# nz0001na/MorphGANformer

Hardware: AMD Instinct MI355X
Metric: latent-projection iters/sec @1024^2, k=17 latents (higher is better)
Workload: dtype f32; 1 GPU; configs[1]: single 1024x1024 face per GPU, Wing+LPIPS(squeeze)+MSE literal-mode projection step, noise_mode=random, seeded synthetic weights/targets/landmarks; k=17, z_dim=32, targets_per_gpu=1, parallelism=pair-sharded x1, graph_replay=True, loss_generator_overlap=True, steps_per_forward=32

## Files before the change

include/mgf.h:

```cpp
#ifndef MGF_H_
#define MGF_H_

#include <stdint.h>

#ifdef __cplusplus
extern "C" {
#endif

typedef void* mgf_stream_t;

enum { MGF_OK = 0, MGF_EINVAL = -1, MGF_EUNSUPPORTED = -2, MGF_ELAUNCH = -3, MGF_ETOOBIG = -4 };
enum { MGF_F32 = 0, MGF_F64 = 1, MGF_F16 = 2 };
enum { MGF_FILTER_SEPARABLE = 2 };
enum { MGF_FILTER_LARGE = 4 };
enum { MGF_ACT_LINEAR = 1, MGF_ACT_RELU = 2, MGF_ACT_LRELU = 3, MGF_ACT_TANH = 4, MGF_ACT_SIGMOID = 5,
       MGF_ACT_ELU = 6, MGF_ACT_SELU = 7, MGF_ACT_SOFTPLUS = 8, MGF_ACT_SWISH = 9,
       MGF_ACT_RELU_POST = 10 };

const char* mgf_last_error(void);
int mgf_version(void);
int mgf_device_ok(void);

int mgf_bias_act(void* y, const void* x, const void* b, const void* xref, const void* yref, const void* dy,
                 int dtype, int64_t numel, int64_t step_b, int64_t size_b,
// ... 70 lines not shown
                              mgf_stream_t stream);
int mgf_conv3x3_winograd3_f32(float* y, const float* x, const float* u, const float* in_scale, const float* out_scale, int32_t n,
                              int32_t cin, int32_t h, int32_t w, int32_t cout, int32_t out_scale_stride, const mgf_epilogue* ep,
                              mgf_stream_t stream);
int mgf_conv3x3_winograd3_slice_f32(float* y, const float* x, const float* u, const float* in_scale, const float* out_scale, int32_t n,
                                    int32_t cin, int32_t h, int32_t w, int32_t cout, int32_t out_scale_stride, int64_t y_batch,
                                    int32_t y_choff, const mgf_epilogue* ep, mgf_stream_t stream);
int mgf_conv1x1_f32(float* y, const float* x, const float* w, const float* in_scale, int32_t n, int32_t cin, int32_t hw, int32_t cout,
                    int32_t cout_pad, int64_t y_batch, int32_t y_choff, const mgf_epilogue* ep, mgf_stream_t stream);
int mgf_conv1x1_force_shape(int32_t channel_blocks);

int mgf_conv3x3s2_few_inputs_f32(float* y, const float* x, const float* w, const float* bias, int32_t n, int32_t cin, int32_t in_h,
                                 int32_t in_w, int32_t cout, int32_t relu, mgf_stream_t stream);
int mgf_tconv3x3s2_few_outputs_f32(float* y, const float* x, const float* wp, int32_t n, int32_t cin, int32_t h, int32_t w, int32_t cout,
                                   int32_t cout_pad, int32_t pitch, int64_t y_plane, int64_t y_batch, mgf_stream_t stream);
int mgf_conv3x3_winograd3_up2res_f32(float* y, const float* x, const float* u, const float* in_scale, const float* out_scale,
                                     const float* residual_low, int32_t n, int32_t cin, int32_t h, int32_t w, int32_t cout,
                                     int32_t out_scale_stride, const mgf_epilogue* ep, mgf_stream_t stream);
int mgf_winograd3_force_shape(int32_t shape);
int mgf_conv3x3_winograd3_rgb_f32(float* rgb_out, const float* x, const float* u, const float* in_scale, const float* out_scale,
                                  const float* rgb_w, const float* rgb_bias, int32_t n, int32_t cin, int32_t h, int32_t w, int32_t cout,
                                  int32_t out_scale_stride, int32_t rgb_channels, mgf_stream_t stream);
int mgf_conv3x3_winograd_f32(float* y, const float* x, const float* u, const float* in_scale, const float* out_scale, int32_t n,
                             int32_t cin, int32_t h, int32_t w, int32_t cout, int32_t out_scale_stride, const mgf_epilogue* ep,
                             mgf_stream_t stream);

int mgf_tconv3x3s2_border_f32(float* t, const float* x, const float* wp, const float* in_scale, const float* out_scale, int32_t n,
                              int32_t cin, int32_t h, int32_t w, int32_t cout, int32_t cout_pad, int64_t t_pitch, int64_t t_plane,
                              int64_t t_batch, int64_t out_scale_stride, mgf_stream_t stream);

int mgf_tconv3x3s2_winograd_f32(float* t, const float* x, const float* u, const float* in_scale, const float* out_scale, int32_t n,
                                int32_t cin, int32_t h, int32_t w, int32_t cout, int32_t pitch, int64_t t_plane, int64_t t_batch,
                                int64_t out_scale_stride, mgf_stream_t stream);
int mgf_tconv_winograd_weights_f32(float* u, const float* w, int32_t cout, int32_t cin, double gain, mgf_stream_t stream);

int mgf_pack_conv_weights(float* wp, float* wsq, const float* w, int32_t cout, int32_t cin, int32_t kh, int32_t kw,
                          int32_t cout_pad, float gain, int32_t flip, mgf_stream_t stream);

typedef struct mgf_style_job {
    const float* aff_w;
    const float* aff_b;
    const float* wsq;
    float* s;
    float* d;
    int32_t cin, cout;
    int32_t w_offset;
    float aff_gain, style_gain;
} mgf_style_job;
int mgf_demod_f32(float* d, const float* s, const float* wsq, int32_t n, int32_t cin, int32_t cout, mgf_stream_t stream);
int mgf_demod_bwd_f32(float* ds, const float* dd, const float* d, const float* s, const float* wsq, int32_t n, int32_t cin, int32_t cout,
                      mgf_stream_t stream);
int mgf_style_demod(const mgf_style_job* job, const float* ws, int64_t ws_stride_n, int32_t n, int32_t wdim, mgf_stream_t stream);
int mgf_style_demod_multi(const mgf_style_job* jobs_dev, int32_t njobs, const float* ws, int64_t ws_stride_n,
                          int32_t n, int32_t wdim, int32_t max_cin, mgf_stream_t stream);

int mgf_duplex_attention(float* y, const float* x, const float* wqc, const float* spos, const float* vwb,
                         int32_t n, int32_t c, int32_t f, int32_t t,
                         const mgf_epilogue* ep, int32_t ep_w, float* probs, int32_t* argmax, mgf_stream_t stream);

int mgf_att_map_upsample_f32(float* out, const float* probs, int32_t n, int32_t side, int32_t t, int32_t out_res, int32_t layer,
                             int32_t n_layers, mgf_stream_t stream);

typedef struct mgf_attn_job {
    const float* wmv;
    const float* bmv;
    float* vwb;
// ... 196 lines not shown
```

morphganformer_amd/_lib.py:

```python
from __future__ import annotations

import ctypes as C
import os

import torch

HERE = os.path.dirname(os.path.abspath(__file__))
LIB_PATH = os.environ.get("MGF_LIB_PATH") or os.path.join(HERE, "libmgf_hip.so")

MGF_F32, MGF_F64, MGF_F16 = 0, 1, 2
ACT_IDS = {"linear": 1, "relu": 2, "lrelu": 3, "tanh": 4, "sigmoid": 5, "elu": 6, "selu": 7, "softplus": 8, "swish": 9,
           "relu_post": 10}
MAX_TAPS = 9

i32, i64, f32, f64, vp = C.c_int32, C.c_int64, C.c_float, C.c_double, C.c_void_p


class Epilogue(C.Structure):
    _fields_ = [("bias", vp), ("noise", vp), ("noise_strength", vp), ("noise_n", i32), ("act", i32), ("alpha", f32),
                ("gain", f32), ("residual", vp)]


class ConvDesc(C.Structure):
    _fields_ = [("n", i32), ("cin", i32), ("in_h", i32), ("in_w", i32), ("cout", i32), ("cout_pad", i32),
# ... 12 lines not shown
    _fields_ = [("aff_w", vp), ("aff_b", vp), ("wsq", vp), ("s", vp), ("d", vp), ("cin", i32), ("cout", i32),
                ("w_offset", i32), ("aff_gain", f32), ("style_gain", f32)]


class AttnJob(C.Structure):
    _fields_ = [("wmv", vp), ("bmv", vp), ("vwb", vp), ("c", i32), ("w_offset", i32)]


class StyleBwdJob(C.Structure):
    _fields_ = [("aff_w", vp), ("wsq", vp), ("s", vp), ("d", vp), ("ds_part", vp), ("dc_part", vp), ("cin", i32), ("cout", i32),
                ("s_chunks", i32), ("d_chunks", i32), ("aff_gain", f32), ("style_gain", f32)]


class AttnGradJob(C.Structure):
    _fields_ = [("dg", vp), ("probs", vp), ("dc", vp), ("cpre", vp), ("part", vp), ("dvwb", vp), ("dc_part", vp), ("c", i32), ("f", i32),
                ("slices", i32), ("nchunk", i32), ("blk_grad", i32), ("blk_dot", i32), ("blk_red", i32), ("pad_", i32)]


class AttnBwdJob(C.Structure):
    _fields_ = [("wmv", vp), ("dvwb", vp), ("c", i32), ("pad_", i32)]


_SIGS = {
    "mgf_last_error": (C.c_char_p, []),
    "mgf_version": (C.c_int, []),
    "mgf_device_ok": (C.c_int, []),
    "mgf_bias_act": (C.c_int, [vp, vp, vp, vp, vp, vp, C.c_int, i64, i64, i64, C.c_int, C.c_int, f32, f32, f32, vp]),
    "mgf_upfirdn2d": (C.c_int, [vp, vp, vp, C.c_int, i32, i32, i32, i32, i64, i64, i64, i64, i32, i32, i64, i64, i64, i64,
                                i32, i32, i32, i32, i32, i32, i32, i32, i32, i32, i32, f32, C.POINTER(Epilogue), vp]),
    "mgf_conv_taps_f32": (C.c_int, [vp, vp, vp, vp, vp, C.POINTER(ConvDesc), C.POINTER(Epilogue), vp]),
    "mgf_conv_taps_bf16x3_f32": (C.c_int, [vp, vp, vp, vp, vp, C.POINTER(ConvDesc), C.POINTER(Epilogue), vp]),
    "mgf_tconv3x3s2_border_f32": (C.c_int, [vp, vp, vp, vp, vp, i32, i32, i32, i32, i32, i32, i64, i64, i64, i64, vp]),
    "mgf_tconv3x3s2_winograd_f32": (C.c_int, [vp, vp, vp, vp, vp, i32, i32, i32, i32, i32, i32, i64, i64, i64, vp]),
    "mgf_tconv_winograd_weights_f32": (C.c_int, [vp, vp, i32, i32, C.c_double, vp]),
    "mgf_winograd_weights_f32": (C.c_int, [vp, vp, i32, i32, f32, vp]),
    "mgf_conv3x3_winograd_f32": (C.c_int, [vp, vp, vp, vp, vp, i32, i32, i32, i32, i32, i32, C.POINTER(Epilogue), vp]),
    "mgf_winograd2_weights_f32": (C.c_int, [vp, vp, i32, i32, f32, vp]),
    "mgf_conv3x3_winograd2_f32": (C.c_int, [vp, vp, vp, vp, vp, i32, i32, i32, i32, i32, i32, C.POINTER(Epilogue), vp]),
    "mgf_conv3x3_winograd2_rgb_f32": (C.c_int, [vp, vp, vp, vp, vp, vp, vp, i32, i32, i32, i32, i32, i32, i32, vp]),
    "mgf_conv3x3_winograd3_f32": (C.c_int, [vp, vp, vp, vp, vp, i32, i32, i32, i32, i32, i32, C.POINTER(Epilogue), vp]),
    "mgf_conv1x1_f32": (C.c_int, [vp, vp, vp, vp, i32, i32, i32, i32, i32, i64, i32, C.POINTER(Epilogue), vp]),
    "mgf_conv3x3s2_few_inputs_f32": (C.c_int, [vp, vp, vp, vp, i32, i32, i32, i32, i32, i32, vp]),
    "mgf_tconv3x3s2_few_outputs_f32": (C.c_int, [vp, vp, vp, i32, i32, i32, i32, i32, i32, i32, i64, i64, vp]),
    "mgf_conv1x1_force_shape": (C.c_int, [i32]),
    "mgf_conv3x3_winograd3_slice_f32": (C.c_int, [vp, vp, vp, vp, vp, i32, i32, i32, i32, i32, i32, i64, i32, C.POINTER(Epilogue), vp]),
    "mgf_conv3x3_winograd3_up2res_f32": (C.c_int, [vp, vp, vp, vp, vp, vp, i32, i32, i32, i32, i32, i32, C.POINTER(Epilogue), vp]),
    "mgf_winograd3_force_shape": (C.c_int, [i32]),
    "mgf_conv3x3_winograd3_rgb_f32": (C.c_int, [vp, vp, vp, vp, vp, vp, vp, i32, i32, i32, i32, i32, i32, i32, vp]),
    "mgf_conv3x3_winograd2_slice_f32": (C.c_int, [vp, vp, vp, vp, vp, i32, i32, i32, i32, i32, i32, i64, i32, C.POINTER(Epilogue), vp]),
    "mgf_pack_conv_weights": (C.c_int, [vp, vp, vp, i32, i32, i32, i32, i32, f32, i32, vp]),
    "mgf_conv_profile_begin": (C.c_int, []),
    "mgf_conv_profile_end": (C.c_int, [C.POINTER(ConvProfRec), i32]),
    "mgf_demod_f32": (C.c_int, [vp, vp, vp, i32, i32, i32, vp]),
    "mgf_demod_bwd_f32": (C.c_int, [vp, vp, vp, vp, vp, i32, i32, i32, vp]),
    "mgf_style_demod": (C.c_int, [C.POINTER(StyleJob), vp, i64, i32, i32, vp]),
    "mgf_style_demod_multi": (C.c_int, [vp, i32, vp, i64, i32, i32, i32, vp]),
    "mgf_duplex_attention": (C.c_int, [vp, vp, vp, vp, vp, i32, i32, i32, i32, C.POINTER(Epilogue), i32, vp, vp, vp]),
    "mgf_att_map_upsample_f32": (C.c_int, [vp, vp, i32, i32, i32, i32, i32, i32, vp]),
    "mgf_attn_values": (C.c_int, [C.POINTER(AttnJob), vp, i64, i64, i32, i32, i32, vp]),
    "mgf_attn_values_multi": (C.c_int, [vp, i32, vp, i64, i64, i32, i32, i32, vp]),
    "mgf_randn_f32": (C.c_int, [vp, i64, C.c_uint64, vp, vp]),
    "mgf_rgb_weights_f32": (C.c_int, [vp, vp, vp, i32, i32, i32, vp]),
    "mgf_torgb_compose_weights_f32": (C.c_int, [vp, vp, vp, vp, vp, vp, i32, i32, i32, i32, vp]),
    "mgf_conv3x3_few_outputs_f32": (C.c_int, [vp, vp, vp, vp, i32, i32, i32, i32, i32, vp]),
    "mgf_mapping_param_floats": (i64, [i32, i32, i32]),
    "mgf_mapping_forward": (C.c_int, [vp, vp, vp, i32, i32, i32, i32, i32, vp]),
# ... 138 lines not shown
```

morphganformer_amd/conv.py:

```python
from __future__ import annotations

import ctypes as C
import os
from dataclasses import dataclass

import torch

from . import _lib


def round_up(v: int, m: int) -> int:
    return (v + m - 1) // m * m


def profile_begin():
    _lib.check(_lib.lib().mgf_conv_profile_begin(), "conv_profile_begin")


def profile_end(max_recs=4096):
    recs = (_lib.ConvProfRec * max_recs)()
    n = _lib.lib().mgf_conv_profile_end(recs, max_recs)
    if n < 0:
        _lib.check(n, "conv_profile_end")
    return [(recs[i].kernel.decode(), recs[i].flops, recs[i].seconds, recs[i].ksplit, recs[i].bytes) for i in range(min(n, max_recs))]
# ... 343 lines not shown

def conv3x3s2_few_inputs(x, w, bias=None, relu=False, out=None):
    _lib.require_gpu(x, w, bias, out)
    cout, cin = w.shape[:2]
    assert tuple(w.shape[2:]) == (3, 3) and cin <= 4 and w.is_contiguous() and w.dtype == torch.float32
    assert x.dtype == torch.float32 and x.is_contiguous() and x.shape[1] == cin
    n, _, h, wd = x.shape
    oh, ow = (h - 3) // 2 + 1, (wd - 3) // 2 + 1
    if out is None:
        out = torch.empty([n, cout, oh, ow], dtype=torch.float32, device=x.device)
    assert out.is_contiguous() and tuple(out.shape) == (n, cout, oh, ow)
    rc = _lib.lib().mgf_conv3x3s2_few_inputs_f32(out.data_ptr(), x.data_ptr(), w.data_ptr(), _lib.ptr(bias), n, cin, h, wd, cout, int(relu),
                                                 _lib.stream_ptr())
    _lib.check(rc, "conv3x3s2_few_inputs")
    return out


def conv3x3_few_outputs(x, w, bias=None, out=None):
    _lib.require_gpu(x, w, bias, out)
    n, cin, h, wd = x.shape
    cout = w.shape[1]
    assert x.dtype == torch.float32 and x.is_contiguous() and w.dtype == torch.float32 and w.is_contiguous()
    assert tuple(w.shape) == (n, cout, cin, 3, 3) and cout <= 4
    if out is None:
        out = torch.empty([n, cout, h, wd], dtype=torch.float32, device=x.device)
    assert out.is_contiguous() and tuple(out.shape) == (n, cout, h, wd)
    _lib.check(_lib.lib().mgf_conv3x3_few_outputs_f32(out.data_ptr(), x.data_ptr(), w.data_ptr(), _lib.ptr(bias), n, cin, h, wd, cout,
                                                      _lib.stream_ptr()), "conv3x3_few_outputs")
    return out


TCONV_WINO = os.environ.get("MGF_TCONV_WINO", "1") != "0"
TCONV_WINO_MIN_WGS = 4096


def tconv_winograd_weights(w: torch.Tensor, gain: float = 1.0) -> torch.Tensor:
    _lib.require_gpu(w)
    w = w.contiguous().float()
    cout, cin, kh, kw = w.shape
    assert (kh, kw) == (3, 3) and cin % 4 == 0
    u = torch.empty([25, cin // 4, cout, 4], dtype=torch.float32, device=w.device)
    _lib.check(_lib.lib().mgf_tconv_winograd_weights_f32(u.data_ptr(), w.data_ptr(), cout, cin, float(gain), _lib.stream_ptr()),
               "tconv_winograd_weights")
    return u


def tconv_winograd_ok(n, cin, h, w, cout, out, bf=None) -> bool:
    return bool(TCONV_WINO and SPLIT_TCONV_BORDER and bf is None and h % 2 == 0 and w % 2 == 0 and min(h, w) >= TCONV_SPLIT_MIN and cin % 4 == 0 and cout % 32 == 0
                and out.shape[3] % 4 == 0 and out.data_ptr() % 16 == 0
                and n * -(-h // 4) * -(-w // 32) * (cout // 32) >= TCONV_WINO_MIN_WGS)


def tconv3x3s2_forward(x, pc: PackedConv, in_scale=None, out_scale=None, out=None, bf=None, wt=None):
    _lib.require_gpu(x, pc.wp, in_scale, out_scale, out, wt)
    assert pc.kh == 3 and pc.kw == 3 and x.dtype == torch.float32 and x.is_contiguous()
    n, cin, h, w = x.shape
    oh, ow = 2 * h + 1, 2 * w + 1
    if out is None:
        out = torch.empty([n, pc.cout, oh, tconv_pitch(w)], dtype=torch.float32, device=x.device)
    pitch = out.shape[3]
    assert out.is_contiguous() and tuple(out.shape) == (n, pc.cout, oh, pitch) and pitch >= ow and pitch % 4 == 0
    if NARROW_CONV and pc.cout <= 4 and in_scale is None and out_scale is None:
        rc = _lib.lib().mgf_tconv3x3s2_few_outputs_f32(out.data_ptr(), x.data_ptr(), pc.wp.data_ptr(), n, cin, h, w, pc.cout, pc.cout_pad,
                                                       pitch, oh * pitch, pc.cout * oh * pitch, _lib.stream_ptr())
        _lib.check(rc, "tconv3x3s2_few_outputs")
        return out[:, :, :, :ow]
    if wt is not None and tconv_winograd_ok(n, cin, h, w, pc.cout, out, bf):
        assert tuple(wt.shape) == (25, cin // 4, pc.cout, 4)
        os_stride = 0 if out_scale is None else out_scale.stride(0) if out_scale.ndim == 2 else 0
        rc = _lib.lib().mgf_tconv3x3s2_winograd_f32(out.data_ptr(), x.data_ptr(), wt.data_ptr(), _lib.ptr(in_scale), _lib.ptr(out_scale), n, cin, h,
                                                    w, pc.cout, pitch, oh * pitch, pc.cout * oh * pitch, os_stride, _lib.stream_ptr())
        _lib.check(rc, "tconv3x3s2_winograd")
        rc = _lib.lib().mgf_tconv3x3s2_border_f32(out.data_ptr(), x.data_ptr(), pc.wp.data_ptr(), _lib.ptr(in_scale), _lib.ptr(out_scale),
                                                  n, cin, h, w, pc.cout, pc.cout_pad, pitch, oh * pitch, pc.cout * oh * pitch, os_stride,
                                                  _lib.stream_ptr())
        _lib.check(rc, "tconv3x3s2_border")
        return out[:, :, :, :ow]
    split = SPLIT_TCONV_BORDER and min(h, w) >= (TCONV_SPLIT_MIN if n >= 4 else max(TCONV_SPLIT_MIN, 128))
    use_bf = bf is not None and split and w % 32 == 0 and cin % 16 == 0
    os_stride = 0 if out_scale is None else out_scale.stride(0) if out_scale.ndim == 2 else 0
    d = _desc(n, cin, h, w, pc.cout, pc.cout_pad, h if split else h + 1, w if split else w + 1, 1, 2, TCONV_TAPS, TCONV_GROUPS,
              [0, 0, 1, 1], [0, 1, 0, 1], oh, ow, pitch, oh * pitch, pc.cout * oh * pitch, 0, os_stride)
    if use_bf:
        rc = _lib.lib().mgf_conv_taps_bf16x3_f32(out.data_ptr(), x.data_ptr(), bf.data_ptr(), _lib.ptr(in_scale), _lib.ptr(out_scale),
                                                 C.byref(d), None, _lib.stream_ptr())
    else:
        rc = _lib.lib().mgf_conv_taps_f32(out.data_ptr(), x.data_ptr(), pc.wp.data_ptr(), _lib.ptr(in_scale), _lib.ptr(out_scale),
                                          C.byref(d), None, _lib.stream_ptr())
    _lib.check(rc, "conv_taps(tconv)")
    if split:
        rc = _lib.lib().mgf_tconv3x3s2_border_f32(out.data_ptr(), x.data_ptr(), pc.wp.data_ptr(), _lib.ptr(in_scale), _lib.ptr(out_scale),
                                                  n, cin, h, w, pc.cout, pc.cout_pad, pitch, oh * pitch, pc.cout * oh * pitch, os_stride,
                                                  _lib.stream_ptr())
        _lib.check(rc, "tconv3x3s2_border")
    return out[:, :, :, :ow]


def upfirdn_into(y, x, f2d, up=1, pad=(0, 0, 0, 0), gain=1.0, flip=False, epilogue=None, separable=False, down=1):
    _lib.require_gpu(x, y, f2d)
    n, c, h, w = x.shape
    fh, fw = f2d.shape
    px0, px1, py0, py1 = pad
# ... 12 lines not shown
```

morphganformer_amd/csrc/conv_taps.hip:

```cpp
#include "mgf_common.h"
#include <vector>

namespace {

typedef float f32x16 __attribute__((ext_vector_type(16)));
typedef __bf16 bf16x8 __attribute__((ext_vector_type(8)));
typedef unsigned u32x4 __attribute__((ext_vector_type(4)));

constexpr int CK = 8;
constexpr int CKB = 16;
template <int WM, int WN> struct Slots {
    static constexpr int XS = WN == 4 ? 20 : (WN == 3 ? 15 : (WN == 1 ? 19 : 11));
    static constexpr int WS = WM == 2 ? 5 : 3;
};

struct Ones { float v[2048]; constexpr Ones() : v() { for (int i = 0; i < 2048; ++i) v[i] = 1.0f; } };
__device__ const Ones g_ones = Ones();

struct ConvParams {
    float* y;
    const float* x;
    const float* wp;
    const float* in_scale;
    const float* out_scale;
// ... 841 lines not shown

void mgf_prof_external_begin(hipStream_t st, const char* name, double flops, double bytes) {
    if (!g_prof_on) return;
    ProfRec r;
    r.name = name; r.wm = r.wn = r.mode = r.pipe = r.nt = 0; r.ksplit = 1; r.flops = flops; r.bytes = bytes;
    (void)hipEventCreate(&r.e0); (void)hipEventCreate(&r.e1);
    (void)hipEventRecord(r.e0, st);
    g_prof.push_back(r);
}
void mgf_prof_external_end(hipStream_t st) {
    if (g_prof_on && !g_prof.empty()) (void)hipEventRecord(g_prof.back().e1, st);
}

extern "C" int mgf_conv_profile_end(mgf_conv_prof_rec* out, int32_t max_recs) {
    g_prof_on = false;
    int n = 0;
    for (auto& r : g_prof) {
        if (hipEventSynchronize(r.e1) != hipSuccess) { mgf_set_error("conv_profile_end: event sync failed"); return MGF_ELAUNCH; }
        float ms = 0.f;
        (void)hipEventElapsedTime(&ms, r.e0, r.e1);
        if (out && n < max_recs) {
            mgf_conv_prof_rec& o = out[n];
            if (r.name) snprintf(o.kernel, sizeof(o.kernel), "%s", r.name);
            else snprintf(o.kernel, sizeof(o.kernel), "conv_taps_kernel<%d, %d, %d, %s, %d, 0>", r.wm, r.wn, r.mode, r.pipe ? "true" : "false", r.nt);
            o.flops = r.flops; o.bytes = r.bytes; o.seconds = ms * 1e-3; o.ksplit = r.ksplit;
        }
        ++n;
        (void)hipEventDestroy(r.e0); (void)hipEventDestroy(r.e1);
    }
    g_prof.clear();
    return n;
}

constexpr int TB_POS = 64, TB_CK = 32, TB_LINE = TB_POS / 2 + 1, TB_LP = TB_LINE + 1;
__global__ __launch_bounds__(256) void tconv_border_kernel(float* t, const float* x, const float* wp, const float* in_scale,
                                                           const float* out_scale, int cin, int h, int w, int cout, int cout_pad,
                                                           int64_t pitch, int64_t plane, int64_t batch, int64_t os_stride, int col_groups) {
    __shared__ float Ws[3][TB_CK][64];
    __shared__ float Xl[TB_CK][TB_LP];
    const int tid = threadIdx.x, n = blockIdx.z, co0 = blockIdx.y * 64;
    const int lane = tid & 63, l31 = lane & 31, half = lane >> 5, wv = __builtin_amdgcn_readfirstlane(tid >> 6);
    const bool col = (int)blockIdx.x < col_groups;
    const int p0 = (col ? blockIdx.x : blockIdx.x - col_groups) * TB_POS;
    const int npos = col ? 2 * h + 1 : 2 * w;
    const int lim = col ? h : w;
    const int tap0 = col ? 2 : 6, tapstep = col ? 3 : 1;
    const float* xn = x + (int64_t)n * cin * h * w;
    const int64_t hw = (int64_t)h * w;
    constexpr int XR = (TB_CK * TB_LINE + 255) / 256, WR = 3 * TB_CK * 64 / 256;
    int xsrc[XR];
#pragma unroll
    for (int r = 0; r < XR; ++r) {
        const int e = tid + 256 * r, jj = e % TB_LINE;
        const int i = p0 / 2 - 1 + jj;
        xsrc[r] = (e < TB_CK * TB_LINE && i >= 0 && i < lim) ? (col ? i * w + (w - 1) : (h - 1) * w + i) : -1;
    }
    float wreg[WR], xreg[XR];
    auto request = [&](int c0) {
#pragma unroll
        for (int r = 0; r < WR; ++r) {
            const int e = tid + 256 * r, co = e & 63, ci = (e >> 6) % TB_CK, k = e / (64 * TB_CK);
            const int cg = c0 + ci < cin ? c0 + ci : cin - 1, cc = co0 + co < cout_pad ? co0 + co : cout_pad - 1;
            wreg[r] = wp[((int64_t)(tap0 + k * tapstep) * cin + cg) * cout_pad + cc];
        }
#pragma unroll
        for (int r = 0; r < XR; ++r) {
            const int e = tid + 256 * r, ci = e / TB_LINE;
            const int cg = c0 + ci < cin ? c0 + ci : cin - 1;
            xreg[r] = xn[cg * hw + (xsrc[r] >= 0 ? xsrc[r] : 0)] * (in_scale ? in_scale[(int64_t)n * cin + cg] : 1.0f);
        }
    };
    f32x16 acc[2];
#pragma unroll
    for (int m = 0; m < 2; ++m)
#pragma unroll
        for (int r = 0; r < 16; ++r) acc[m][r] = 0.f;
    request(0);
    for (int c0 = 0; c0 < cin; c0 += TB_CK) {
        __syncthreads();
#pragma unroll
        for (int r = 0; r < WR; ++r) {
            const int e = tid + 256 * r, co = e & 63, ci = (e >> 6) % TB_CK, k = e / (64 * TB_CK);
            Ws[k][ci][co] = c0 + ci < cin ? wreg[r] : 0.f;
        }
#pragma unroll
        for (int r = 0; r < XR; ++r) {
            const int e = tid + 256 * r, jj = e % TB_LINE, ci = e / TB_LINE;
            if (e < TB_CK * TB_LINE) Xl[ci][jj] = (c0 + ci < cin && xsrc[r] >= 0) ? xreg[r] : 0.f;
        }
        __syncthreads();
        if (c0 + TB_CK < cin) request(c0 + TB_CK);
        if (wv < 2) {
#pragma unroll 8
            for (int ci = 0; ci < TB_CK; ++ci)
                acc[0] = __builtin_amdgcn_mfma_f32_32x32x2f32(Ws[2 * half][ci][wv * 32 + l31], Xl[ci][l31 + 1 - half], acc[0], 0, 0, 0);
        } else if (wv == 2) {
#pragma unroll 8
            for (int cp = 0; cp < TB_CK / 2; ++cp) {
                const int ci = 2 * cp + half;
                const float bv = Xl[ci][l31 + 1];
                acc[0] = __builtin_amdgcn_mfma_f32_32x32x2f32(Ws[1][ci][l31], bv, acc[0], 0, 0, 0);
                acc[1] = __builtin_amdgcn_mfma_f32_32x32x2f32(Ws[1][ci][32 + l31], bv, acc[1], 0, 0, 0);
            }
        }
    }
    if (wv > 2) return;
    const int q = p0 + 2 * l31 + (wv == 2 ? 1 : 0);
    if (q >= npos) return;
    const int oy = col ? q : 2 * h, ox = col ? 2 * w : q;
    float* tn = t + (int64_t)n * batch + (int64_t)oy * pitch + ox;
#pragma unroll
    for (int m = 0; m < 2; ++m) {
        if (m == 1 && wv != 2) break;
        const int cb = wv == 2 ? m : wv;
#pragma unroll
        for (int r = 0; r < 16; ++r) {
            const int co = co0 + cb * 32 + (r & 3) + 8 * (r >> 2) + 4 * half;
            if (co < cout) tn[(int64_t)co * plane] = acc[m][r] * (out_scale ? out_scale[(int64_t)n * os_stride + co] : 1.0f);
        }
    }
}

extern "C" int mgf_tconv3x3s2_border_f32(float* t, const float* x, const float* wp, const float* in_scale, const float* out_scale,
                                         int32_t n, int32_t cin, int32_t h, int32_t w, int32_t cout, int32_t cout_pad, int64_t t_pitch,
                                         int64_t t_plane, int64_t t_batch, int64_t out_scale_stride, mgf_stream_t stream) {
    MGF_REQUIRE(t && x && wp && n >= 1 && n <= 65535 && cin >= 1 && h >= 1 && w >= 1 && cout >= 1 && cout_pad >= cout, MGF_EINVAL,
                "tconv3x3s2_border: bad arguments");
    MGF_REQUIRE(t_pitch >= 2 * w + 1 && t_plane >= (int64_t)(2 * h + 1) * t_pitch, MGF_EINVAL, "tconv3x3s2_border: output pitch/plane too small");
    const int col_groups = (int)mgf_cdiv(2 * h + 1, TB_POS), row_groups = (int)mgf_cdiv(2 * w, TB_POS);
    hipLaunchKernelGGL(tconv_border_kernel, dim3(col_groups + row_groups, (unsigned)mgf_cdiv(cout, 64), n), dim3(256), 0, (hipStream_t)stream,
                       t, x, wp, in_scale, out_scale, cin, h, w, cout, cout_pad, t_pitch, t_plane, t_batch, out_scale_stride, col_groups);
    MGF_CHECK_LAUNCH("tconv3x3s2_border");
    return MGF_OK;
}

extern "C" int mgf_pack_conv_weights(float* wp, float* wsq, const float* w, int32_t cout, int32_t cin, int32_t kh, int32_t kw,
                                     int32_t cout_pad, float gain, int32_t flip, mgf_stream_t stream) {
    MGF_REQUIRE(wp && w, MGF_EINVAL, "pack_conv_weights: null pointer");
    MGF_REQUIRE(cout >= 1 && cin >= 1 && kh >= 1 && kw >= 1 && kh * kw <= MGF_MAX_TAPS, MGF_EINVAL, "pack_conv_weights: bad shape");
    MGF_REQUIRE(cout_pad >= cout && cout_pad % 32 == 0, MGF_EINVAL, "pack_conv_weights: cout_pad must be a multiple of 32 >= cout");
    const int64_t total = (int64_t)kh * kw * cin * cout_pad;
    hipLaunchKernelGGL(pack_weights_kernel, dim3(mgf_stream_grid(total, 256, 4)), dim3(256), 0, (hipStream_t)stream, wp, wsq, w,
                       cout, cin, kh, kw, cout_pad, gain, flip);
    MGF_CHECK_LAUNCH("pack_conv_weights");
    return MGF_OK;
}

static int conv_taps_dispatch(float* y, const float* x, const float* wp, const void* wb, const float* in_scale, const float* out_scale,
                              const mgf_conv_desc* dd, const mgf_epilogue* ep, mgf_stream_t stream) {
    MGF_REQUIRE(x && (wp || wb) && dd && (y || dd->rgb_out), MGF_EINVAL, "conv_taps: null pointer");
    const mgf_conv_desc& d = *dd;
    MGF_REQUIRE(d.n >= 1 && d.cin >= 1 && d.cout >= 1 && d.in_h >= 1 && d.in_w >= 1, MGF_EINVAL, "conv_taps: bad shape");
    MGF_REQUIRE(d.cout_pad >= d.cout && d.cout_pad % 32 == 0, MGF_EINVAL, "conv_taps: cout_pad must be a multiple of 32 >= cout");
// ... 148 lines not shown
```

morphganformer_amd/csrc/mgf_common.h:

```cpp
#pragma once
#include <hip/hip_runtime.h>
#include <stdint.h>
#include <stdio.h>
#include <stdarg.h>
#include "../../include/mgf.h"

#define MGF_WAVE 64
#define MGF_NUM_CU 256
#define MGF_NUM_XCD 8

void mgf_set_error(const char* fmt, ...);

#define MGF_REQUIRE(cond, code, ...)            \
    do {                                         \
        if (!(cond)) {                           \
            mgf_set_error(__VA_ARGS__);          \
            return (code);                       \
        }                                        \
    } while (0)

#define MGF_CHECK_LAUNCH(name)                                                        \
    do {                                                                              \
        hipError_t e_ = hipGetLastError();                                            \
        if (e_ != hipSuccess) {                                                       \
// ... 10 lines not shown
#else
static inline constexpr const char* mgf_knob(const char*) { return nullptr; }
#endif

static inline int mgf_stream_grid(int64_t work_items, int block, int per_thread) {
    int64_t g = mgf_cdiv(work_items, (int64_t)block * per_thread);
    int64_t cap = (int64_t)MGF_NUM_CU * 8;
    if (g > cap) g = cap;
    if (g < 1) g = 1;
    return (int)g;
}

void mgf_prof_external_begin(hipStream_t st, const char* name, double flops, double bytes);
void mgf_prof_external_end(hipStream_t st);

int mgf_wino3_batch_invariant_f32(float* y, const float* x, const float* u, int32_t n, int32_t cin, int32_t h, int32_t w, int32_t cout,
                                  const mgf_epilogue* ep, mgf_stream_t stream);
int mgf_wino3_batch_invariant_masked_f32(float* y, const float* x, const float* u, const float* mask, int32_t n, int32_t c, int32_t h, int32_t w,
                                         int32_t ring, float slope, mgf_stream_t stream);

#ifdef __HIPCC__
template <typename T>
__device__ __forceinline__ T wave_sum(T v) {
#pragma unroll
    for (int o = 32; o > 0; o >>= 1) v += __shfl_xor(v, o, 64);
    return v;
}
template <typename T>
__device__ __forceinline__ T wave_max(T v) {
#pragma unroll
    for (int o = 32; o > 0; o >>= 1) { T u = __shfl_xor(v, o, 64); v = u > v ? u : v; }
    return v;
}
#endif
```

morphganformer_amd/csrc/wino_tconv.hip:

```cpp
#include "mgf_common.h"
#include <algorithm>
#include <type_traits>

namespace {

typedef float f32x16 __attribute__((ext_vector_type(16)));
typedef float v2f __attribute__((ext_vector_type(2)));

constexpr int WTCK = 4;
constexpr int WTFW = 34;
constexpr int WTFH = 5;
constexpr int WTFP = WTFH * WTFW;
constexpr int WTNP = 25;
constexpr int WTXS = 14;
__constant__ float wt_ones[WTCK] = {1.f, 1.f, 1.f, 1.f};

struct WinoTParams {
    float* t;
    const float* x;
    const float* u;
    const float* in_scale;
    const float* out_scale;
    int n, cin, h, w, cout, os_stride, pitch;
    int tiles_x, tiles_y, co_tiles;
    int xcd_per;
    int64_t t_plane, t_batch;
};

__global__ __launch_bounds__(256, 2) void wino_tconv_kernel(WinoTParams p) {
    constexpr int CST = 256, RAW = WTCK * CST;
    extern __shared__ float lds[];
    float* const raw0 = lds;
    float* const raw1 = raw0 + RAW;
    const int tid = threadIdx.x, lane = tid & 63;
    const int a = __builtin_amdgcn_readfirstlane(tid >> 6);
    const int l31 = lane & 31, half = lane >> 5;
    const int tx = l31 & 15, ty = l31 >> 4;

    int b_ = blockIdx.x;
    if (p.xcd_per > 0) {
        b_ = (b_ & 7) * p.xcd_per + (b_ >> 3);
        if (b_ >= p.n * p.tiles_x * p.tiles_y * p.co_tiles) return;
    }
    const int cot = b_ % p.co_tiles; b_ /= p.co_tiles;
    const int ptx = b_ % p.tiles_x; b_ /= p.tiles_x;
    const int pty = b_ % p.tiles_y;
    const int n = b_ / p.tiles_y;
    const int co0 = cot * 32, iy0 = pty * 4, ix0 = ptx * 32;
    const int plane = p.h * p.w;
    const float* xn = p.x + (int64_t)n * p.cin * plane;
    const float* sc = p.in_scale ? p.in_scale + (int64_t)n * p.cin : nullptr;
    const int nck = p.cin / WTCK;

    const __amdgpu_buffer_rsrc_t rx = __builtin_amdgcn_make_buffer_rsrc((void*)xn, 0, p.cin * plane * 4, 0x00020000);
    const __amdgpu_buffer_rsrc_t ru = __builtin_amdgcn_make_buffer_rsrc((void*)p.u, 0, WTNP * p.cin * p.cout * 4, 0x00020000);
    const __amdgpu_buffer_rsrc_t rnull = __builtin_amdgcn_make_buffer_rsrc((void*)p.u, 0, 0, 0x00020000);
    unsigned xoff;
    {
        const int r = tid / WTFW, q = tid - r * WTFW;
        const int iy = iy0 - 1 + r, ix = ix0 - 1 + q;
        xoff = (tid < WTFP && iy >= 0 && iy < p.h && ix >= 0 && ix < p.w) ? (unsigned)(iy * p.w + ix) * 4u : 0xFFFFFFF0u;
    }
    const unsigned aoff = (unsigned)(((co0 + l31) * WTCK + half * 2) * 4);
    const int upos = nck * p.cout * WTCK * 4;
    const int ubase_row = 5 * a * upos, ubase_col = (20 + a) * upos, ubase_sh = 24 * upos + (a & 1) * 4;

    float xr[WTCK];
    auto load_x = [&](float (&dst)[WTCK], int c0, bool live = true) {
        const __amdgpu_buffer_rsrc_t r = live ? rx : rnull;
#pragma unroll
        for (int j = 0; j < WTCK; ++j) dst[j] = __builtin_bit_cast(float, __builtin_amdgcn_raw_buffer_load_b32(r, xoff, (c0 + j) * plane * 4, 0));
    };
// ... 187 lines not shown
        double t[5][3];
#pragma unroll
        for (int v = 0; v < 3; ++v) {
            const double g0 = g[v], g1 = g[3 + v], g2 = g[6 + v];
            t[0][v] = g2;
            t[1][v] = g0 + g2;
            t[2][v] = g0;
            t[3][v] = g1;
            t[4][v] = g1;
        }
        const int cl = ci & 3, slot = 2 * (cl & 1) + (cl >> 1);
        const int64_t pl = (int64_t)cin * cout;
        float* dst = u + (((int64_t)(ci >> 2)) * cout + co) * 4 + slot;
#pragma unroll
        for (int r = 0; r < 5; ++r) {
            const double o[5] = {t[r][2], t[r][0] + t[r][2], t[r][0], t[r][1], t[r][1]};
#pragma unroll
            for (int c = 0; c < 5; ++c) dst[(5 * r + c) * pl] = (float)(o[c] * gain);
        }
    }
}

}

extern "C" int mgf_tconv_winograd_weights_f32(float* u, const float* w, int32_t cout, int32_t cin, double gain, mgf_stream_t stream) {
    MGF_REQUIRE(u && w && cout >= 1 && cin >= 1, MGF_EINVAL, "tconv_winograd_weights: bad arguments");
    MGF_REQUIRE(cin % WTCK == 0, MGF_EUNSUPPORTED, "tconv_winograd_weights: cin must be a multiple of %d (got %d)", WTCK, cin);
    hipLaunchKernelGGL(wino_tconv_weights_kernel, dim3(mgf_stream_grid((int64_t)cout * cin, 256, 1)), dim3(256), 0, (hipStream_t)stream, u, w, cout,
                       cin, gain);
    MGF_CHECK_LAUNCH("tconv_winograd_weights");
    return MGF_OK;
}

extern "C" int mgf_tconv3x3s2_winograd_f32(float* t, const float* x, const float* u, const float* in_scale, const float* out_scale, int32_t n,
                                           int32_t cin, int32_t h, int32_t w, int32_t cout, int32_t pitch, int64_t t_plane, int64_t t_batch,
                                           int64_t out_scale_stride, mgf_stream_t stream) {
    MGF_REQUIRE(t && x && u && n >= 1 && cin >= 1 && cout >= 1 && h >= 2 && w >= 2, MGF_EINVAL, "tconv3x3s2_winograd: bad arguments");
    MGF_REQUIRE(cin % WTCK == 0 && cout % 32 == 0, MGF_EUNSUPPORTED, "tconv3x3s2_winograd: cin must be a multiple of %d and cout of 32 (got %d, %d)",
                WTCK, cin, cout);
    MGF_REQUIRE(h % 2 == 0 && w % 2 == 0, MGF_EUNSUPPORTED, "tconv3x3s2_winograd: even map sides only (got %dx%d)", h, w);
    MGF_REQUIRE(pitch >= 2 * w + 1 && pitch % 4 == 0 && t_plane >= (int64_t)(2 * h + 1) * pitch && t_plane % 4 == 0 && t_batch % 4 == 0 &&
                    t_batch >= (int64_t)cout * t_plane, MGF_EINVAL, "tconv3x3s2_winograd: bad workspace layout");
    MGF_REQUIRE(((uintptr_t)t % 16) == 0 && ((uintptr_t)u % 16) == 0, MGF_EINVAL, "tconv3x3s2_winograd: t and u must be 16-byte aligned");
    MGF_REQUIRE((int64_t)cin * h * w <= INT32_MAX / 4 && (int64_t)WTNP * cin * cout <= INT32_MAX / 4 && (int64_t)cout * t_plane <= INT32_MAX / 4,
                MGF_ETOOBIG, "tconv3x3s2_winograd: one sample / the weight planes must stay below 2 GiB (32-bit buffer offsets)");
    WinoTParams p{};
    p.t = t; p.x = x; p.u = u; p.in_scale = in_scale; p.out_scale = out_scale;
    p.n = n; p.cin = cin; p.h = h; p.w = w; p.cout = cout; p.os_stride = (int)out_scale_stride; p.pitch = pitch;
    p.t_plane = t_plane; p.t_batch = t_batch;
    p.tiles_x = (int)mgf_cdiv(w, 32);
    p.tiles_y = (int)mgf_cdiv(h, 4);
    p.co_tiles = cout / 32;
    int64_t blocks = (int64_t)n * p.tiles_x * p.tiles_y * p.co_tiles;
    MGF_REQUIRE(blocks <= INT32_MAX - 8, MGF_ETOOBIG, "tconv3x3s2_winograd: too many workgroups");
    p.xcd_per = 0;
    if ((int64_t)WTNP * cin * cout * 4 <= (4 << 20) && blocks >= 16) {
        p.xcd_per = (int)((blocks + 7) / 8);
        blocks = (int64_t)p.xcd_per * 8;
    }
    const size_t lds = std::max<size_t>((size_t)2 * WTCK * 256, (size_t)WTXS * 16 * 64) * sizeof(float);
    static bool attr_set = false;
    if (!attr_set) {
        hipError_t e = hipFuncSetAttribute((const void*)wino_tconv_kernel, hipFuncAttributeMaxDynamicSharedMemorySize, 65536);
        if (e != hipSuccess) { mgf_set_error("tconv3x3s2_winograd: cannot raise dynamic LDS: %s", hipGetErrorString(e)); return MGF_ELAUNCH; }
        attr_set = true;
    }
    mgf_prof_external_begin((hipStream_t)stream, "wino_tconv_kernel", 2.0 * 9 * cin * (double)cout * h * w * n,
                            4.0 * ((double)n * cin * h * w + 9.0 * cin * cout + (double)n * cout * 4.0 * h * w));
    hipLaunchKernelGGL(wino_tconv_kernel, dim3((unsigned)blocks), dim3(256), lds, (hipStream_t)stream, p);
    mgf_prof_external_end((hipStream_t)stream);
    MGF_CHECK_LAUNCH("tconv3x3s2_winograd");
    return MGF_OK;
}
```

Before: 789.9 iters/s.

## Fold tconv border kernel into the Winograd tconv launch as extra workgroups

Moves the transposed-conv border computation into a shared device function and dispatches it from the Winograd tconv kernel as a prefix range of workgroups, so maps of side 128 and up need one launch instead of two. This removes a separate kernel launch and its tail/serialization gap, and lets border work overlap with the main Winograd tiles. The cost is a larger LDS reservation and register pressure in the fused kernel, which could reduce occupancy of the main Winograd path.

```diff
diff --git a/include/mgf.h b/include/mgf.h
--- a/include/mgf.h
+++ b/include/mgf.h
@@ -126,6 +126,9 @@
 int mgf_tconv3x3s2_winograd_f32(float* t, const float* x, const float* u, const float* in_scale, const float* out_scale, int32_t n,
                                 int32_t cin, int32_t h, int32_t w, int32_t cout, int32_t pitch, int64_t t_plane, int64_t t_batch,
                                 int64_t out_scale_stride, mgf_stream_t stream);
+int mgf_tconv3x3s2_winograd_full_f32(float* t, const float* x, const float* u, const float* wp, const float* in_scale, const float* out_scale,
+                                     int32_t n, int32_t cin, int32_t h, int32_t w, int32_t cout, int32_t cout_pad, int32_t pitch,
+                                     int64_t t_plane, int64_t t_batch, int64_t out_scale_stride, mgf_stream_t stream);
 int mgf_tconv_winograd_weights_f32(float* u, const float* w, int32_t cout, int32_t cin, double gain, mgf_stream_t stream);
 
 int mgf_pack_conv_weights(float* wp, float* wsq, const float* w, int32_t cout, int32_t cin, int32_t kh, int32_t kw,
diff --git a/morphganformer_amd/_lib.py b/morphganformer_amd/_lib.py
--- a/morphganformer_amd/_lib.py
+++ b/morphganformer_amd/_lib.py
@@ -68,6 +68,7 @@
     "mgf_conv_taps_bf16x3_f32": (C.c_int, [vp, vp, vp, vp, vp, C.POINTER(ConvDesc), C.POINTER(Epilogue), vp]),
     "mgf_tconv3x3s2_border_f32": (C.c_int, [vp, vp, vp, vp, vp, i32, i32, i32, i32, i32, i32, i64, i64, i64, i64, vp]),
     "mgf_tconv3x3s2_winograd_f32": (C.c_int, [vp, vp, vp, vp, vp, i32, i32, i32, i32, i32, i32, i64, i64, i64, vp]),
+    "mgf_tconv3x3s2_winograd_full_f32": (C.c_int, [vp, vp, vp, vp, vp, vp, i32, i32, i32, i32, i32, i32, i32, i64, i64, i64, vp]),
     "mgf_tconv_winograd_weights_f32": (C.c_int, [vp, vp, i32, i32, C.c_double, vp]),
     "mgf_winograd_weights_f32": (C.c_int, [vp, vp, i32, i32, f32, vp]),
     "mgf_conv3x3_winograd_f32": (C.c_int, [vp, vp, vp, vp, vp, i32, i32, i32, i32, i32, i32, C.POINTER(Epilogue), vp]),
diff --git a/morphganformer_amd/conv.py b/morphganformer_amd/conv.py
--- a/morphganformer_amd/conv.py
+++ b/morphganformer_amd/conv.py
@@ -399,6 +399,8 @@
 
 TCONV_WINO = os.environ.get("MGF_TCONV_WINO", "1") != "0"
 TCONV_WINO_MIN_WGS = 4096
+TCONV_FOLD_BORDER = os.environ.get("MGF_TCONV_FOLD_BORDER", "1") != "0"
+TCONV_FOLD_MIN_SIDE = 128
 
 
 def tconv_winograd_weights(w: torch.Tensor, gain: float = 1.0) -> torch.Tensor:
@@ -435,6 +437,12 @@
     if wt is not None and tconv_winograd_ok(n, cin, h, w, pc.cout, out, bf):
         assert tuple(wt.shape) == (25, cin // 4, pc.cout, 4)
         os_stride = 0 if out_scale is None else out_scale.stride(0) if out_scale.ndim == 2 else 0
+        if TCONV_FOLD_BORDER and min(h, w) >= TCONV_FOLD_MIN_SIDE:
+            rc = _lib.lib().mgf_tconv3x3s2_winograd_full_f32(out.data_ptr(), x.data_ptr(), wt.data_ptr(), pc.wp.data_ptr(), _lib.ptr(in_scale),
+                                                             _lib.ptr(out_scale), n, cin, h, w, pc.cout, pc.cout_pad, pitch, oh * pitch,
+                                                             pc.cout * oh * pitch, os_stride, _lib.stream_ptr())
+            _lib.check(rc, "tconv3x3s2_winograd_full")
+            return out[:, :, :, :ow]
         rc = _lib.lib().mgf_tconv3x3s2_winograd_f32(out.data_ptr(), x.data_ptr(), wt.data_ptr(), _lib.ptr(in_scale), _lib.ptr(out_scale), n, cin, h,
                                                     w, pc.cout, pitch, oh * pitch, pc.cout * oh * pitch, os_stride, _lib.stream_ptr())
         _lib.check(rc, "tconv3x3s2_winograd")
diff --git a/morphganformer_amd/csrc/conv_taps.hip b/morphganformer_amd/csrc/conv_taps.hip
--- a/morphganformer_amd/csrc/conv_taps.hip
+++ b/morphganformer_amd/csrc/conv_taps.hip
@@ -897,93 +897,12 @@
     return n;
 }
 
-constexpr int TB_POS = 64, TB_CK = 32, TB_LINE = TB_POS / 2 + 1, TB_LP = TB_LINE + 1;
 __global__ __launch_bounds__(256) void tconv_border_kernel(float* t, const float* x, const float* wp, const float* in_scale,
                                                            const float* out_scale, int cin, int h, int w, int cout, int cout_pad,
                                                            int64_t pitch, int64_t plane, int64_t batch, int64_t os_stride, int col_groups) {
-    __shared__ float Ws[3][TB_CK][64];
-    __shared__ float Xl[TB_CK][TB_LP];
-    const int tid = threadIdx.x, n = blockIdx.z, co0 = blockIdx.y * 64;
-    const int lane = tid & 63, l31 = lane & 31, half = lane >> 5, wv = __builtin_amdgcn_readfirstlane(tid >> 6);
-    const bool col = (int)blockIdx.x < col_groups;
-    const int p0 = (col ? blockIdx.x : blockIdx.x - col_groups) * TB_POS;
-    const int npos = col ? 2 * h + 1 : 2 * w;
-    const int lim = col ? h : w;
-    const int tap0 = col ? 2 : 6, tapstep = col ? 3 : 1;
-    const float* xn = x + (int64_t)n * cin * h * w;
-    const int64_t hw = (int64_t)h * w;
-    constexpr int XR = (TB_CK * TB_LINE + 255) / 256, WR = 3 * TB_CK * 64 / 256;
-    int xsrc[XR];
-#pragma unroll
-    for (int r = 0; r < XR; ++r) {
-        const int e = tid + 256 * r, jj = e % TB_LINE;
-        const int i = p0 / 2 - 1 + jj;
-        xsrc[r] = (e < TB_CK * TB_LINE && i >= 0 && i < lim) ? (col ? i * w + (w - 1) : (h - 1) * w + i) : -1;
-    }
-    float wreg[WR], xreg[XR];
-    auto request = [&](int c0) {
-#pragma unroll
-        for (int r = 0; r < WR; ++r) {
-            const int e = tid + 256 * r, co = e & 63, ci = (e >> 6) % TB_CK, k = e / (64 * TB_CK);
-            const int cg = c0 + ci < cin ? c0 + ci : cin - 1, cc = co0 + co < cout_pad ? co0 + co : cout_pad - 1;
-            wreg[r] = wp[((int64_t)(tap0 + k * tapstep) * cin + cg) * cout_pad + cc];
-        }
-#pragma unroll
-        for (int r = 0; r < XR; ++r) {
-            const int e = tid + 256 * r, ci = e / TB_LINE;
-            const int cg = c0 + ci < cin ? c0 + ci : cin - 1;
-            xreg[r] = xn[cg * hw + (xsrc[r] >= 0 ? xsrc[r] : 0)] * (in_scale ? in_scale[(int64_t)n * cin + cg] : 1.0f);
-        }
-    };
-    f32x16 acc[2];
-#pragma unroll
-    for (int m = 0; m < 2; ++m)
-#pragma unroll
-        for (int r = 0; r < 16; ++r) acc[m][r] = 0.f;
-    request(0);
-    for (int c0 = 0; c0 < cin; c0 += TB_CK) {
-        __syncthreads();
-#pragma unroll
-        for (int r = 0; r < WR; ++r) {
-            const int e = tid + 256 * r, co = e & 63, ci = (e >> 6) % TB_CK, k = e / (64 * TB_CK);
-            Ws[k][ci][co] = c0 + ci < cin ? wreg[r] : 0.f;
-        }
-#pragma unroll
-        for (int r = 0; r < XR; ++r) {
-            const int e = tid + 256 * r, jj = e % TB_LINE, ci = e / TB_LINE;
-            if (e < TB_CK * TB_LINE) Xl[ci][jj] = (c0 + ci < cin && xsrc[r] >= 0) ? xreg[r] : 0.f;
-        }
-        __syncthreads();
-        if (c0 + TB_CK < cin) request(c0 + TB_CK);
-        if (wv < 2) {
-#pragma unroll 8
-            for (int ci = 0; ci < TB_CK; ++ci)
-                acc[0] = __builtin_amdgcn_mfma_f32_32x32x2f32(Ws[2 * half][ci][wv * 32 + l31], Xl[ci][l31 + 1 - half], acc[0], 0, 0, 0);
-        } else if (wv == 2) {
-#pragma unroll 8
-            for (int cp = 0; cp < TB_CK / 2; ++cp) {
-                const int ci = 2 * cp + half;
-                const float bv = Xl[ci][l31 + 1];
-                acc[0] = __builtin_amdgcn_mfma_f32_32x32x2f32(Ws[1][ci][l31], bv, acc[0], 0, 0, 0);
-                acc[1] = __builtin_amdgcn_mfma_f32_32x32x2f32(Ws[1][ci][32 + l31], bv, acc[1], 0, 0, 0);
-            }
-        }
-    }
-    if (wv > 2) return;
-    const int q = p0 + 2 * l31 + (wv == 2 ? 1 : 0);
-    if (q >= npos) return;
-    const int oy = col ? q : 2 * h, ox = col ? 2 * w : q;
-    float* tn = t + (int64_t)n * batch + (int64_t)oy * pitch + ox;
-#pragma unroll
-    for (int m = 0; m < 2; ++m) {
-        if (m == 1 && wv != 2) break;
-        const int cb = wv == 2 ? m : wv;
-#pragma unroll
-        for (int r = 0; r < 16; ++r) {
-            const int co = co0 + cb * 32 + (r & 3) + 8 * (r >> 2) + 4 * half;
-            if (co < cout) tn[(int64_t)co * plane] = acc[m][r] * (out_scale ? out_scale[(int64_t)n * os_stride + co] : 1.0f);
-        }
-    }
+    __shared__ float smem[TB_LDS_FLOATS];
+    mgf_tconv_border_item(smem, blockIdx.x, blockIdx.y * 64, blockIdx.z, t, x, wp, in_scale, out_scale, cin, h, w, cout, cout_pad, pitch, plane,
+                          batch, os_stride, col_groups);
 }
 
 extern "C" int mgf_tconv3x3s2_border_f32(float* t, const float* x, const float* wp, const float* in_scale, const float* out_scale,
diff --git a/morphganformer_amd/csrc/mgf_common.h b/morphganformer_amd/csrc/mgf_common.h
--- a/morphganformer_amd/csrc/mgf_common.h
+++ b/morphganformer_amd/csrc/mgf_common.h
@@ -66,4 +66,96 @@
     for (int o = 32; o > 0; o >>= 1) { T u = __shfl_xor(v, o, 64); v = u > v ? u : v; }
     return v;
 }
+
+constexpr int TB_POS = 64, TB_CK = 32, TB_LINE = TB_POS / 2 + 1, TB_LP = TB_LINE + 1;
+constexpr int TB_LDS_FLOATS = 3 * TB_CK * 64 + TB_CK * TB_LP;
+__device__ __forceinline__ void mgf_tconv_border_item(float* smem, int item, int co0, int n, float* t, const float* x, const float* wp,
+                                                      const float* in_scale, const float* out_scale, int cin, int h, int w, int cout,
+                                                      int cout_pad, int64_t pitch, int64_t plane, int64_t batch, int64_t os_stride,
+                                                      int col_groups) {
+    typedef float f32x16 __attribute__((ext_vector_type(16)));
+    float (*const Ws)[TB_CK][64] = reinterpret_cast<float (*)[TB_CK][64]>(smem);
+    float (*const Xl)[TB_LP] = reinterpret_cast<float (*)[TB_LP]>(smem + 3 * TB_CK * 64);
+    const int tid = threadIdx.x;
+    const int lane = tid & 63, l31 = lane & 31, half = lane >> 5, wv = __builtin_amdgcn_readfirstlane(tid >> 6);
+    const bool col = item < col_groups;
+    const int p0 = (col ? item : item - col_groups) * TB_POS;
+    const int npos = col ? 2 * h + 1 : 2 * w;
+    const int lim = col ? h : w;
+    const int tap0 = col ? 2 : 6, tapstep = col ? 3 : 1;
+    const float* xn = x + (int64_t)n * cin * h * w;
+    const int64_t hw = (int64_t)h * w;
+    constexpr int XR = (TB_CK * TB_LINE + 255) / 256, WR = 3 * TB_CK * 64 / 256;
+    int xsrc[XR];
+#pragma unroll
+    for (int r = 0; r < XR; ++r) {
+        const int e = tid + 256 * r, jj = e % TB_LINE;
+        const int i = p0 / 2 - 1 + jj;
+        xsrc[r] = (e < TB_CK * TB_LINE && i >= 0 && i < lim) ? (col ? i * w + (w - 1) : (h - 1) * w + i) : -1;
+    }
+    float wreg[WR], xreg[XR];
+    auto request = [&](int c0) {
+#pragma unroll
+        for (int r = 0; r < WR; ++r) {
+            const int e = tid + 256 * r, co = e & 63, ci = (e >> 6) % TB_CK, k = e / (64 * TB_CK);
+            const int cg = c0 + ci < cin ? c0 + ci : cin - 1, cc = co0 + co < cout_pad ? co0 + co : cout_pad - 1;
+            wreg[r] = wp[((int64_t)(tap0 + k * tapstep) * cin + cg) * cout_pad + cc];
+        }
+#pragma unroll
+        for (int r = 0; r < XR; ++r) {
+            const int e = tid + 256 * r, ci = e / TB_LINE;
+            const int cg = c0 + ci < cin ? c0 + ci : cin - 1;
+            xreg[r] = xn[cg * hw + (xsrc[r] >= 0 ? xsrc[r] : 0)] * (in_scale ? in_scale[(int64_t)n * cin + cg] : 1.0f);
+        }
+    };
+    f32x16 acc[2];
+#pragma unroll
+    for (int m = 0; m < 2; ++m)
+#pragma unroll
+        for (int r = 0; r < 16; ++r) acc[m][r] = 0.f;
+    request(0);
+    for (int c0 = 0; c0 < cin; c0 += TB_CK) {
+        __syncthreads();
+#pragma unroll
+        for (int r = 0; r < WR; ++r) {
+            const int e = tid + 256 * r, co = e & 63, ci = (e >> 6) % TB_CK, k = e / (64 * TB_CK);
+            Ws[k][ci][co] = c0 + ci < cin ? wreg[r] : 0.f;
+        }
+#pragma unroll
+        for (int r = 0; r < XR; ++r) {
+            const int e = tid + 256 * r, jj = e % TB_LINE, ci = e / TB_LINE;
+            if (e < TB_CK * TB_LINE) Xl[ci][jj] = (c0 + ci < cin && xsrc[r] >= 0) ? xreg[r] : 0.f;
+        }
+        __syncthreads();
+        if (c0 + TB_CK < cin) request(c0 + TB_CK);
+        if (wv < 2) {
+#pragma unroll 8
+            for (int ci = 0; ci < TB_CK; ++ci)
+                acc[0] = __builtin_amdgcn_mfma_f32_32x32x2f32(Ws[2 * half][ci][wv * 32 + l31], Xl[ci][l31 + 1 - half], acc[0], 0, 0, 0);
+        } else if (wv == 2) {
+#pragma unroll 8
+            for (int cp = 0; cp < TB_CK / 2; ++cp) {
+                const int ci = 2 * cp + half;
+                const float bv = Xl[ci][l31 + 1];
+                acc[0] = __builtin_amdgcn_mfma_f32_32x32x2f32(Ws[1][ci][l31], bv, acc[0], 0, 0, 0);
+                acc[1] = __builtin_amdgcn_mfma_f32_32x32x2f32(Ws[1][ci][32 + l31], bv, acc[1], 0, 0, 0);
+            }
+        }
+    }
+    if (wv > 2) return;
+    const int q = p0 + 2 * l31 + (wv == 2 ? 1 : 0);
+    if (q >= npos) return;
+    const int oy = col ? q : 2 * h, ox = col ? 2 * w : q;
+    float* tn = t + (int64_t)n * batch + (int64_t)oy * pitch + ox;
+#pragma unroll
+    for (int m = 0; m < 2; ++m) {
+        if (m == 1 && wv != 2) break;
+        const int cb = wv == 2 ? m : wv;
+#pragma unroll
+        for (int r = 0; r < 16; ++r) {
+            const int co = co0 + cb * 32 + (r & 3) + 8 * (r >> 2) + 4 * half;
+            if (co < cout) tn[(int64_t)co * plane] = acc[m][r] * (out_scale ? out_scale[(int64_t)n * os_stride + co] : 1.0f);
+        }
+    }
+}
 #endif
diff --git a/morphganformer_amd/csrc/wino_tconv.hip b/morphganformer_amd/csrc/wino_tconv.hip
--- a/morphganformer_amd/csrc/wino_tconv.hip
+++ b/morphganformer_amd/csrc/wino_tconv.hip
@@ -25,6 +25,8 @@
     int tiles_x, tiles_y, co_tiles;
     int xcd_per;
     int64_t t_plane, t_batch;
+    const float* wp;
+    int cout_pad, border_wgs, border_items, border_gx, border_gy, col_groups;
 };
 
 __global__ __launch_bounds__(256, 2) void wino_tconv_kernel(WinoTParams p) {
@@ -37,7 +39,15 @@
     const int l31 = lane & 31, half = lane >> 5;
     const int tx = l31 & 15, ty = l31 >> 4;
 
-    int b_ = blockIdx.x;
+    if ((int)blockIdx.x < p.border_wgs) {
+        int b = blockIdx.x;
+        if (b >= p.border_items) return;
+        const int item = b % p.border_gx; b /= p.border_gx;
+        mgf_tconv_border_item(lds, item, (b % p.border_gy) * 64, b / p.border_gy, p.t, p.x, p.wp, p.in_scale, p.out_scale, p.cin, p.h, p.w, p.cout,
+                              p.cout_pad, p.pitch, p.t_plane, p.t_batch, p.os_stride, p.col_groups);
+        return;
+    }
+    int b_ = blockIdx.x - p.border_wgs;
     if (p.xcd_per > 0) {
         b_ = (b_ & 7) * p.xcd_per + (b_ >> 3);
         if (b_ >= p.n * p.tiles_x * p.tiles_y * p.co_tiles) return;
@@ -291,18 +301,18 @@
     return MGF_OK;
 }
 
-extern "C" int mgf_tconv3x3s2_winograd_f32(float* t, const float* x, const float* u, const float* in_scale, const float* out_scale, int32_t n,
-                                           int32_t cin, int32_t h, int32_t w, int32_t cout, int32_t pitch, int64_t t_plane, int64_t t_batch,
-                                           int64_t out_scale_stride, mgf_stream_t stream) {
-    MGF_REQUIRE(t && x && u && n >= 1 && cin >= 1 && cout >= 1 && h >= 2 && w >= 2, MGF_EINVAL, "tconv3x3s2_winograd: bad arguments");
-    MGF_REQUIRE(cin % WTCK == 0 && cout % 32 == 0, MGF_EUNSUPPORTED, "tconv3x3s2_winograd: cin must be a multiple of %d and cout of 32 (got %d, %d)",
-                WTCK, cin, cout);
-    MGF_REQUIRE(h % 2 == 0 && w % 2 == 0, MGF_EUNSUPPORTED, "tconv3x3s2_winograd: even map sides only (got %dx%d)", h, w);
+static int launch_wino_tconv(const char* what, float* t, const float* x, const float* u, const float* wp, const float* in_scale, const float* out_scale,
+                             int32_t n, int32_t cin, int32_t h, int32_t w, int32_t cout, int32_t cout_pad, int32_t pitch, int64_t t_plane,
+                             int64_t t_batch, int64_t out_scale_stride, mgf_stream_t stream) {
+    MGF_REQUIRE(t && x && u && n >= 1 && cin >= 1 && cout >= 1 && h >= 2 && w >= 2, MGF_EINVAL, "%s: bad arguments", what);
+    MGF_REQUIRE(cin % WTCK == 0 && cout % 32 == 0, MGF_EUNSUPPORTED, "%s: cin must be a multiple of %d and cout of 32 (got %d, %d)", what, WTCK, cin,
+                cout);
+    MGF_REQUIRE(h % 2 == 0 && w % 2 == 0, MGF_EUNSUPPORTED, "%s: even map sides only (got %dx%d)", what, h, w);
     MGF_REQUIRE(pitch >= 2 * w + 1 && pitch % 4 == 0 && t_plane >= (int64_t)(2 * h + 1) * pitch && t_plane % 4 == 0 && t_batch % 4 == 0 &&
-                    t_batch >= (int64_t)cout * t_plane, MGF_EINVAL, "tconv3x3s2_winograd: bad workspace layout");
-    MGF_REQUIRE(((uintptr_t)t % 16) == 0 && ((uintptr_t)u % 16) == 0, MGF_EINVAL, "tconv3x3s2_winograd: t and u must be 16-byte aligned");
+                    t_batch >= (int64_t)cout * t_plane, MGF_EINVAL, "%s: bad workspace layout", what);
+    MGF_REQUIRE(((uintptr_t)t % 16) == 0 && ((uintptr_t)u % 16) == 0, MGF_EINVAL, "%s: t and u must be 16-byte aligned", what);
     MGF_REQUIRE((int64_t)cin * h * w <= INT32_MAX / 4 && (int64_t)WTNP * cin * cout <= INT32_MAX / 4 && (int64_t)cout * t_plane <= INT32_MAX / 4,
-                MGF_ETOOBIG, "tconv3x3s2_winograd: one sample / the weight planes must stay below 2 GiB (32-bit buffer offsets)");
+                MGF_ETOOBIG, "%s: one sample / the weight planes must stay below 2 GiB (32-bit buffer offsets)", what);
     WinoTParams p{};
     p.t = t; p.x = x; p.u = u; p.in_scale = in_scale; p.out_scale = out_scale;
     p.n = n; p.cin = cin; p.h = h; p.w = w; p.cout = cout; p.os_stride = (int)out_scale_stride; p.pitch = pitch;
@@ -311,23 +321,51 @@
     p.tiles_y = (int)mgf_cdiv(h, 4);
     p.co_tiles = cout / 32;
     int64_t blocks = (int64_t)n * p.tiles_x * p.tiles_y * p.co_tiles;
-    MGF_REQUIRE(blocks <= INT32_MAX - 8, MGF_ETOOBIG, "tconv3x3s2_winograd: too many workgroups");
     p.xcd_per = 0;
     if ((int64_t)WTNP * cin * cout * 4 <= (4 << 20) && blocks >= 16) {
         p.xcd_per = (int)((blocks + 7) / 8);
         blocks = (int64_t)p.xcd_per * 8;
     }
-    const size_t lds = std::max<size_t>((size_t)2 * WTCK * 256, (size_t)WTXS * 16 * 64) * sizeof(float);
+    if (wp) {
+        MGF_REQUIRE(cout_pad >= cout, MGF_EINVAL, "%s: cout_pad < cout", what);
+        p.wp = wp; p.cout_pad = cout_pad;
+        p.col_groups = (int)mgf_cdiv(2 * h + 1, TB_POS);
+        p.border_gx = p.col_groups + (int)mgf_cdiv(2 * w, TB_POS);
+        p.border_gy = (int)mgf_cdiv(cout, 64);
+        const int64_t items = (int64_t)p.border_gx * p.border_gy * n;
+        MGF_REQUIRE(items <= INT32_MAX / 2, MGF_ETOOBIG, "%s: too many workgroups", what);
+        p.border_items = (int)items;
+        p.border_wgs = (int)(mgf_cdiv(items, 8) * 8);
+        blocks += p.border_wgs;
+    }
+    MGF_REQUIRE(blocks <= INT32_MAX - 8, MGF_ETOOBIG, "%s: too many workgroups", what);
+    const size_t lds = std::max<size_t>({(size_t)2 * WTCK * 256, (size_t)WTXS * 16 * 64, (size_t)TB_LDS_FLOATS}) * sizeof(float);
     static bool attr_set = false;
     if (!attr_set) {
         hipError_t e = hipFuncSetAttribute((const void*)wino_tconv_kernel, hipFuncAttributeMaxDynamicSharedMemorySize, 65536);
-        if (e != hipSuccess) { mgf_set_error("tconv3x3s2_winograd: cannot raise dynamic LDS: %s", hipGetErrorString(e)); return MGF_ELAUNCH; }
+        if (e != hipSuccess) { mgf_set_error("%s: cannot raise dynamic LDS: %s", what, hipGetErrorString(e)); return MGF_ELAUNCH; }
         attr_set = true;
     }
     mgf_prof_external_begin((hipStream_t)stream, "wino_tconv_kernel", 2.0 * 9 * cin * (double)cout * h * w * n,
                             4.0 * ((double)n * cin * h * w + 9.0 * cin * cout + (double)n * cout * 4.0 * h * w));
     hipLaunchKernelGGL(wino_tconv_kernel, dim3((unsigned)blocks), dim3(256), lds, (hipStream_t)stream, p);
     mgf_prof_external_end((hipStream_t)stream);
-    MGF_CHECK_LAUNCH("tconv3x3s2_winograd");
+    MGF_CHECK_LAUNCH(what);
     return MGF_OK;
 }
+
+extern "C" int mgf_tconv3x3s2_winograd_f32(float* t, const float* x, const float* u, const float* in_scale, const float* out_scale, int32_t n,
+                                           int32_t cin, int32_t h, int32_t w, int32_t cout, int32_t pitch, int64_t t_plane, int64_t t_batch,
+                                           int64_t out_scale_stride, mgf_stream_t stream) {
+    return launch_wino_tconv("tconv3x3s2_winograd", t, x, u, nullptr, in_scale, out_scale, n, cin, h, w, cout, cout, pitch, t_plane, t_batch,
+                             out_scale_stride, stream);
+}
+
+extern "C" int mgf_tconv3x3s2_winograd_full_f32(float* t, const float* x, const float* u, const float* wp, const float* in_scale,
+                                                const float* out_scale, int32_t n, int32_t cin, int32_t h, int32_t w, int32_t cout,
+                                                int32_t cout_pad, int32_t pitch, int64_t t_plane, int64_t t_batch, int64_t out_scale_stride,
+                                                mgf_stream_t stream) {
+    MGF_REQUIRE(wp, MGF_EINVAL, "tconv3x3s2_winograd_full: bad arguments");
+    return launch_wino_tconv("tconv3x3s2_winograd_full", t, x, u, wp, in_scale, out_scale, n, cin, h, w, cout, cout_pad, pitch, t_plane, t_batch,
+                             out_scale_stride, stream);
+}
```

Result: no change. 789.3 iters/s (-0.1%).
